# opendilab/LightZero

Hardware: NVIDIA H100
Metric: MCTS simulations/sec (batched search+infer) (higher is better)
Workload: dtype f32 (fp16x2-split tensor MMAs, fp32 accumulate)

## Files before the change

lightzero_b200/csrc/conv_tc.cu:

```cuda
#include <math.h>
#include <stdlib.h>
#include <string.h>

#include <algorithm>

#include "conv_tc.cuh"
#include "tc_ptx.cuh"

namespace lz {

constexpr int kCvConsumers = 256, kCvThreads = kCvConsumers + 32;
constexpr int kCvStages = 4;

struct CvBars {
    uint64_t full[kCvStages], empty[kCvStages];
    uint64_t in_full;
};

struct CvGeom {
    int nbands, rin, m_lo, mcount, NT, PR;
    size_t plane, part, phase, in_bytes, tap_bytes, smem;
};

__host__ __device__ inline CvGeom cv_geom(const ConvTc &p)
// ... 47 lines not shown
        mbar_init(&bars->in_full, 1);
        fence_mbar_init();
    }
    __syncthreads();

    if (warp == kCvConsumers / 32) {
        if (lane == 0) {
            const int grow0 = rin0 + 1;
            const int ncopy = min(g.rin, p.in.plane_rows - grow0);
            const uint32_t bytes = (uint32_t)ncopy * 16u;
            mbar_expect_tx(&bars->in_full, bytes * (uint32_t)(nimg * p.in.nphase * 2 * kg_in));
            for (int k = 0; k < nimg; ++k)
                for (int f = 0; f < p.in.nphase; ++f)
                    for (int part = 0; part < 2; ++part)
                        for (int kg = 0; kg < kg_in; ++kg) {
                            const unsigned char *src = p.in.base + (size_t)(img0 + k) * p.in.img_stride + f * p.in.phase_stride +
                                                       part * p.in.part_stride + ((size_t)kg * p.in.plane_rows + grow0) * 16;
                            unsigned char *dst = in_s + f * g.phase + part * g.part + kg * g.plane + (size_t)k * g.rin * 16;
                            bulk_g2s(dst, src, bytes, &bars->in_full);
                        }
            for (int n = 0; n < 9 * g.NT; ++n) {
                const int st = n % nstages, tap = n % 9;
                if (n >= nstages) mbar_wait(&bars->empty[st], ((n / nstages) - 1) & 1);
                mbar_expect_tx(&bars->full[st], (uint32_t)g.tap_bytes);
                bulk_g2s(ring + st * g.tap_bytes, p.w + (size_t)tap * g.tap_bytes, (uint32_t)g.tap_bytes, &bars->full[st]);
            }
        }
        return;
    }

    const int wg = warp >> 2;
    const uint32_t plane16 = (uint32_t)(g.plane >> 4);
    const uint64_t a_desc0 = make_desc(smem_u32(in_s), plane16, 8);
    const uint64_t b_desc0 = make_desc(smem_u32(ring), 2 * N, 8);
    const uint32_t b_lo16 = (uint32_t)N;
    const uint32_t a_lo16 = (uint32_t)(g.part >> 4);
    const int nks = kg_in / 2;
    const int yend = min(y0 + p.band_h, H);
    const int qc = 2 * (lane & 3);
    mbar_wait(&bars->in_full, 0);
    for (int t = 0; t < g.NT; ++t) {
        float acc[N / 2];
#pragma unroll
        for (int i = 0; i < N / 2; ++i) acc[i] = 0.0f;
        for (int tap = 0; tap < 9; ++tap) {
            const int n = t * 9 + tap, st = n % nstages;
            mbar_wait(&bars->full[st], (n / nstages) & 1);
            const uint64_t b0 = b_desc0 + (uint64_t)((st * g.tap_bytes) >> 4);
            const uint64_t a0 = a_desc0 + (uint64_t)((p.tap_phase[tap] * g.phase) >> 4) + (uint64_t)(g.m_lo + p.tap_shift[tap] + t * 128 + wg * 64);
            wg_fence();
            for (int ks = 0; ks < nks; ++ks) {
                wgmma_f16<N>(acc, a0 + ks * 2 * plane16, b0 + ks * 4 * N);
                if (npass == 3) {
                    wgmma_f16<N>(acc, a0 + ks * 2 * plane16, b0 + b_lo16 + ks * 4 * N);
                    wgmma_f16<N>(acc, a0 + a_lo16 + ks * 2 * plane16, b0 + ks * 4 * N);
                }
            }
            wg_commit();
            if (tap > 0) {
                wg_wait<1>();
                __syncwarp();
                if (lane == 0) mbar_arrive(&bars->empty[(n - 1) % nstages]);
            }
        }
        wg_wait<0>();
        __syncwarp();
        if (lane == 0) mbar_arrive(&bars->empty[(t * 9 + 8) % nstages]);

#pragma unroll
        for (int hr = 0; hr < 2; ++hr) {
            const int m = g.m_lo + t * 128 + wg * 64 + 16 * (warp & 3) + (lane >> 2) + 8 * hr;
            const int k = m / g.rin;
            const int rho = rin0 + (m - k * g.rin);
            const int yy = rho / pitch - 1, xx = rho - (yy + 1) * pitch;
            const bool in_band = (k < nimg) && (rho >= pitch) && (yy >= y0) && (yy < yend);
            const bool valid = in_band && (xx < W);
#pragma unroll
            for (int j = 0; j < N / 8; ++j) {
                const int col = 8 * j + qc;
                const int grp = (N == 128) ? (col >> 6) : 0;
                const int c = col - grp * 64;
                const Tcl &o = p.out[grp];
                const bool relu = p.relu[grp] != 0;
                size_t obase = 0;
                bool do_write = in_band;
                if (in_band) {
                    if (o.nphase == 1) {
                        obase = (size_t)(img0 + k) * o.img_stride + (size_t)(rho + 1) * 16;
                    } else if (valid) {
                        const int ph = (yy & 1) * 2 + (xx & 1);
                        const int rho2 = ((yy >> 1) + 1) * o.pitch + (xx >> 1);
                        obase = (size_t)(img0 + k) * o.img_stride + ph * o.phase_stride + (size_t)(rho2 + 1) * 16;
                    } else {
                        do_write = false;
                    }
                }
                float v0 = fmaf(acc[4 * j + 2 * hr], __ldg(p.scale + col), __ldg(p.shift + col));
                float v1 = fmaf(acc[4 * j + 2 * hr + 1], __ldg(p.scale + col + 1), __ldg(p.shift + col + 1));
                if (p.res.base && grp == 0 && valid) {
                    const unsigned char *rp = p.res.base + (size_t)(img0 + k) * p.res.img_stride +
                                              ((size_t)(c >> 3) * p.res.plane_rows + rho + 1) * 16 + (c & 7) * 2;
                    const float2 a = __half22float2(*reinterpret_cast<const __half2 *>(rp));
                    const float2 b = __half22float2(*reinterpret_cast<const __half2 *>(rp + p.res.part_stride));
                    v0 += a.x + b.x;
                    v1 += a.y + b.y;
                }
                v0 = valid ? (relu ? fmaxf(v0, 0.0f) : v0) : 0.0f;
                v1 = valid ? (relu ? fmaxf(v1, 0.0f) : v1) : 0.0f;
                if (do_write) {
                    unsigned char *op = o.base + obase + (size_t)(c >> 3) * o.plane_rows * 16 + (c & 7) * 2;
                    store_split2(op, op + o.part_stride, v0, v1);
                }
            }
        }
    }
}

__device__ __forceinline__ void tcl_load8(const Tcl &t, int img, int kg, int rho, float (&v)[8])
{
    const unsigned char *pp = t.base + (size_t)img * t.img_stride + ((size_t)kg * t.plane_rows + rho + 1) * 16;
    const uint4 rh = __ldg(reinterpret_cast<const uint4 *>(pp));
    const uint4 rl = __ldg(reinterpret_cast<const uint4 *>(pp + t.part_stride));
    const __half2 *hh = reinterpret_cast<const __half2 *>(&rh), *hl = reinterpret_cast<const __half2 *>(&rl);
#pragma unroll
    for (int j = 0; j < 4; ++j) {
        const float2 a = __half22float2(hh[j]), b = __half22float2(hl[j]);
        v[2 * j] = a.x + b.x;
        v[2 * j + 1] = a.y + b.y;
    }
}

__global__ void k_pool_tcl(Tcl in, Tcl out, float *out_nchw, int B, int Hout)
{
    const int kgs = in.C / 8;
    const size_t n = (size_t)B * kgs * Hout * Hout;
    for (size_t i = blockIdx.x * (size_t)blockDim.x + threadIdx.x; i < n; i += (size_t)gridDim.x * blockDim.x) {
        const int xo = (int)(i % Hout), yo = (int)((i / Hout) % Hout);
        const int kg = (int)((i / ((size_t)Hout * Hout)) % kgs), img = (int)(i / ((size_t)Hout * Hout * kgs));
        float s[8];
#pragma unroll
        for (int j = 0; j < 8; ++j) s[j] = 0.0f;
#pragma unroll
        for (int ky = 0; ky < 3; ++ky) {
            const int yy = 2 * yo + ky - 1;
            if (yy < 0 || yy >= in.H) continue;
#pragma unroll
            for (int kx = 0; kx < 3; ++kx) {
                const int xx = 2 * xo + kx - 1;
                if (xx < 0 || xx >= in.W) continue;
                float v[8];
                tcl_load8(in, img, kg, (yy + 1) * in.pitch + xx, v);
#pragma unroll
                for (int j = 0; j < 8; ++j) s[j] += v[j];
            }
        }
#pragma unroll
        for (int j = 0; j < 8; ++j) s[j] = s[j] / 9.0f;
        if (out_nchw) {
#pragma unroll
            for (int j = 0; j < 8; ++j) out_nchw[((size_t)img * in.C + kg * 8 + j) * Hout * Hout + yo * Hout + xo] = s[j];
        } else {
            unsigned char *op = out.base + (size_t)img * out.img_stride + ((size_t)kg * out.plane_rows + (yo + 1) * out.pitch + xo + 1) * 16;
            store_split8(op, op + out.part_stride, s);
        }
    }
}

int conv_tc_prepare_launch()
{
    const int big = 227 * 1024;
    LZ_CUDA_CHECK(cudaFuncSetAttribute(k_conv_tc<32>, cudaFuncAttributeMaxDynamicSharedMemorySize, big));
    LZ_CUDA_CHECK(cudaFuncSetAttribute(k_conv_tc<64>, cudaFuncAttributeMaxDynamicSharedMemorySize, big));
    LZ_CUDA_CHECK(cudaFuncSetAttribute(k_conv_tc<128>, cudaFuncAttributeMaxDynamicSharedMemorySize, big));
    return LZ_OK;
}

int conv_tc_launch(const ConvTc &p, cudaStream_t s)
{
    const CvGeom g = cv_geom(p);
    LZ_REQUIRE(g.smem <= 227 * 1024, LZ_EINVAL, "conv_tc: band needs %zu B shared memory", g.smem);
    LZ_REQUIRE(g.tap_bytes <= 16384 && (p.in.C % 16) == 0, LZ_EINVAL, "conv_tc: unsupported channel counts");
    const int groups = (p.B + p.G - 1) / p.G;
    const int grid = groups * g.nbands;
    switch (p.N) {
        case 32: k_conv_tc<32><<<grid, kCvThreads, g.smem, s>>>(p); break;
        case 64: k_conv_tc<64><<<grid, kCvThreads, g.smem, s>>>(p); break;
        case 128: k_conv_tc<128><<<grid, kCvThreads, g.smem, s>>>(p); break;
        default: LZ_REQUIRE(false, LZ_EINVAL, "conv_tc: N must be 32, 64 or 128");
    }
    LZ_KERNEL_CHECK();
    return LZ_OK;
}

size_t conv_tc_packed_bytes(int cin, int ncols) { return (size_t)9 * 2 * (cin / 8) * ncols * 16; }

float conv_tc_pack(const float *w, int cin, int cout, int ncols, int col0, unsigned char *dst)
{
    float mx = 0.0f;
    for (size_t i = 0; i < (size_t)cout * cin * 9; ++i) mx = std::max(mx, fabsf(w[i]));
    int e = 0;
    if (mx > 0.0f) frexpf(mx, &e);
    const float scale = ldexpf(1.0f, 13 - e);
    const size_t tap_halves = (size_t)2 * (cin / 8) * ncols * 8, part_halves = (size_t)ncols * 8;
    __half *h = reinterpret_cast<__half *>(dst);
    for (int t = 0; t < 9; ++t)
        for (int co = 0; co < cout; ++co)
            for (int ci = 0; ci < cin; ++ci) {
                const float sv = w[((size_t)co * cin + ci) * 9 + t] * scale;
                const __half hi = __float2half_rn(sv);
                const __half lo = __float2half_rn(sv - __half2float(hi));
                const size_t off = (size_t)t * tap_halves + ((size_t)(ci / 8) * 2 * ncols + col0 + co) * 8 + (ci % 8);
                h[off] = hi;
                h[off + part_halves] = lo;
            }
    return scale;
}

int pool_tcl_launch(const Tcl &in, const Tcl &out, int B, cudaStream_t s)
{
    const size_t n = (size_t)B * (in.C / 8) * out.H * out.W;
    k_pool_tcl<<<(int)std::min<size_t>((n + 255) / 256, kNumSMs * 32), 256, 0, s>>>(in, out, nullptr, B, out.H);
    LZ_KERNEL_CHECK();
    return LZ_OK;
}

int pool_tcl_to_nchw_launch(const Tcl &in, float *out, int B, int Hout, cudaStream_t s)
{
    const size_t n = (size_t)B * (in.C / 8) * Hout * Hout;
    Tcl dummy = in;
    k_pool_tcl<<<(int)std::min<size_t>((n + 255) / 256, kNumSMs * 32), 256, 0, s>>>(in, dummy, out, B, Hout);
    LZ_KERNEL_CHECK();
    return LZ_OK;
}

}
```

lightzero_b200/csrc/conv_tc.cuh:

```cuda
#pragma once
#include "lz_common.cuh"

namespace lz {

struct Tcl {
    unsigned char *base;
    size_t img_stride, phase_stride, part_stride;
    int plane_rows;
    int C, H, W, pitch;
    int nphase;
};

inline Tcl make_tcl(unsigned char *base, int C, int H, int W, int nphase)
{
    Tcl t;
    t.base = base; t.C = C; t.H = H; t.W = W; t.pitch = W + 1; t.nphase = nphase;
    t.plane_rows = (H + 2) * (W + 1) + 2;
    t.part_stride = (size_t)(C / 8) * t.plane_rows * 16;
    t.phase_stride = 2 * t.part_stride;
    t.img_stride = t.phase_stride * nphase;
    return t;
}
inline size_t tcl_bytes(int B, int C, int H, int W, int nphase)
{
    return (size_t)B * nphase * 2 * (C / 8) * ((size_t)(H + 2) * (W + 1) + 2) * 16;
}

struct ConvTc {
    Tcl in;
    Tcl out[2];
    Tcl res;
    const unsigned char *w;
    const float *scale, *shift;
    int tap_phase[9], tap_shift[9];
    int relu[2];
    int N;
    int G, band_h;
    int stages;
    int B, npass;
};

int conv_tc_prepare_launch();
int conv_tc_launch(const ConvTc &p, cudaStream_t s);
float conv_tc_pack(const float *w_torch, int cin, int cout, int ncols, int col0, unsigned char *dst);
size_t conv_tc_packed_bytes(int cin, int ncols);

int pool_tcl_launch(const Tcl &in, const Tcl &out, int B, cudaStream_t s);
int pool_tcl_to_nchw_launch(const Tcl &in, float *out, int B, int Hout, cudaStream_t s);

}
```

lightzero_b200/csrc/model.cu:

```cuda
#include <math.h>
#include <string.h>

#include <algorithm>

#include "model.cuh"
#include "tc_ptx.cuh"

namespace lz {

constexpr int kActFloats = kC * kP;
constexpr int kHFlatMax = 16 * kP;
constexpr int kKpad = 608;

template <int W>
__device__ __forceinline__ void heads_and_outputs(const NetDev &net, float *actA, float *actB, float *hrew,
                                                  float *wstage, bool with_reward, int B, float *o_reward,
                                                  float *o_value, float *o_policy, float *o_reward_logits,
                                                  float *o_value_logits)
{
    const int w = threadIdx.x >> 5, lane = threadIdx.x & 31;
    const int A = net.A, Apad = (A + 31) & ~31;
    float *lg_rew = actB;
    float *lg_val = actB + W * kKpad;
    float *lg_pol = actB + 2 * W * kKpad;
// ... 374 lines not shown
        }
        return tc_launch(m->tc_rec, t, s);
    }
    switch (pick_W(io.B)) {
        case 8: return launch_recurrent<8>(m->net, io, s);
        case 4: return launch_recurrent<4>(m->net, io, s);
        case 2: return launch_recurrent<2>(m->net, io, s);
        default: return launch_recurrent<1>(m->net, io, s);
    }
}

static int launch_convg(const ConvG &L, const float *in, float *out, const float *res, int relu, int B, cudaStream_t s,
                        const Tcl *tcl = nullptr, const uint8_t *in_u8 = nullptr)
{
    Tcl t;
    memset(&t, 0, sizeof(t));
    if (tcl) t = *tcl;
    const int cic = std::min(8, L.cin);
    const int rows_out_max = std::min(L.hout, 127 / L.wout + 2);
    const int nrows_max = (rows_out_max - 1) * L.stride + 3;
    const int pitch = L.win + 2;
    const size_t smem = ((((size_t)cic * nrows_max * pitch + 3) & ~(size_t)3) + (size_t)cic * 288) * sizeof(float);
    dim3 grid(ceil_div(L.hout * L.wout, 128), L.cout / 32, B);
    LZ_REQUIRE(smem <= 200 * 1024, LZ_EINVAL, "conv tower stage needs %zu B shared memory", smem);
    if (L.stride == 1) k_conv3x3_generic<1><<<grid, 128, smem, s>>>(L, in, out, res, relu, cic, nrows_max, t, in_u8);
    else k_conv3x3_generic<2><<<grid, 128, smem, s>>>(L, in, out, res, relu, cic, nrows_max, t, in_u8);
    LZ_KERNEL_CHECK();
    return LZ_OK;
}

static int launch_pool(const float *in, float *out, int planes, int hin, int hout, cudaStream_t s)
{
    const size_t n = (size_t)planes * hout * hout;
    int blocks = (int)std::min<size_t>((n + 255) / 256, kNumSMs * 16);
    k_avgpool3s2<<<blocks, 256, 0, s>>>(in, out, planes, hin, hin, hout, hout);
    LZ_KERNEL_CHECK();
    return LZ_OK;
}

static int reserve_tc_skip(lz_model *m, int B)
{
    if (m->kind != 0 || B <= m->tc_skip_B) return LZ_OK;
    ++m->generation;
    cudaFree(m->tc_skip);
    m->tc_skip = nullptr; m->tc_skip_B = 0;
    int rc = dev_alloc(&m->tc_skip, (size_t)kActFloats * B);
    if (rc != LZ_OK) return rc;
    m->tc_skip_B = B;
    return LZ_OK;
}

int model_reserve(lz_model *m, int B)
{
    {
        int rc = reserve_tc_skip(m, B);
        if (rc != LZ_OK) return rc;
    }
    if (m->kind == 0 && m->cfg.efficientzero && B > m->ez_B) {
        ++m->generation;
        cudaFree(m->ez_feat); cudaFree(m->ez_htmp);
        m->ez_feat = m->ez_htmp = nullptr;
        int rc = dev_alloc(&m->ez_feat, (size_t)B * m->cfg.reward_head_channels * kP);
        if (rc == LZ_OK) rc = dev_alloc(&m->ez_htmp, (size_t)B * m->cfg.lstm_hidden_size);
        if (rc != LZ_OK) return rc;
        m->ez_B = B;
    }
    if (m->kind == 1 || B <= m->ws_B) return LZ_OK;
    ++m->generation;
    size_t per_root = 0;
    for (const ConvG &L : m->tower) per_root = std::max(per_root, (size_t)L.cout * L.hout * L.wout);
    per_root = std::max(per_root, (size_t)kActFloats);
    for (int i = 0; i < 3; ++i) {
        if (m->ws[i]) cudaFree(m->ws[i]);
        m->ws[i] = nullptr;
        int rc = dev_alloc(&m->ws[i], per_root * B);
        if (rc != LZ_OK) return rc;
    }
    m->ws_floats = per_root * B;
    m->ws_B = B;
    {
        const int h1 = m->tower[0].hout, h2 = m->tower[3].hout, h3 = (h2 - 1) / 2 + 1, c2 = kC / 2;
        const size_t bT = tcl_bytes(B, c2, h1, h1, 1), bT2 = tcl_bytes(B, c2, h1 / 2, h1 / 2, 4);
        const size_t bU = tcl_bytes(B, kC, h2, h2, 1), bV = tcl_bytes(B, kC, h3, h3, 1);
        const size_t total = 2 * bT + bT2 + 3 * bU + 3 * bV;
        if (m->tws) cudaFree(m->tws);
        m->tws = nullptr;
        int rc = dev_alloc(&m->tws, total);
        if (rc != LZ_OK) return rc;
        LZ_CUDA_CHECK(cudaMemset(m->tws, 0, total));
        m->tws_bytes = total;
        unsigned char *q = m->tws;
        m->T0 = make_tcl(q, c2, h1, h1, 1); q += bT;
        m->T1 = make_tcl(q, c2, h1, h1, 1); q += bT;
        m->T2 = make_tcl(q, c2, h1 / 2, h1 / 2, 4); q += bT2;
        m->U0 = make_tcl(q, kC, h2, h2, 1); q += bU;
        m->U1 = make_tcl(q, kC, h2, h2, 1); q += bU;
        m->U2 = make_tcl(q, kC, h2, h2, 1); q += bU;
        m->V0 = make_tcl(q, kC, h3, h3, 1); q += bV;
        m->V1 = make_tcl(q, kC, h3, h3, 1); q += bV;
        m->V2 = make_tcl(q, kC, h3, h3, 1); q += bV;
    }
    return LZ_OK;
}

static void pick_band(ConvTc &p)
{
    const int H = p.in.H, pitch = p.in.pitch, kg = p.in.C / 8;
    double best = -1.0;
    int best_h = 1, best_g = 1, best_st = 4;
    for (int G = 1; G <= 4; ++G)
        for (int bh = (G > 1 ? H : 1); bh <= H; ++bh)
            for (int st = 2; st <= 4; st += 2) {
                const int rin = (bh + 2) * pitch + 2, mcount = (G - 1) * rin + bh * pitch, NT = (mcount + 127) / 128;
                int PR = pitch + 1 + NT * 128 + pitch + 2;
                if (PR < G * rin) PR = G * rin;
                const size_t smem = (((size_t)PR * 16 * kg * 2 * p.in.nphase + 127) & ~(size_t)127) + st * (size_t)2 * kg * p.N * 16 + 1024;
                if (smem > 227 * 1024) continue;
                const int nb = (H + bh - 1) / bh;
                double score = (double)(G * H * (pitch - 1)) / ((double)nb * NT * 128);
                if (p.N <= 64 && smem <= 113 * 1024) score *= 1.35;
                score *= (st == 4) ? 1.0 : 0.97;
                if (score > best + 1e-9) { best = score; best_h = bh; best_g = G; best_st = st; }
            }
    p.band_h = best_h;
    p.G = best_g;
    p.stages = best_st;
}

static int tower_tc_run(lz_model *m, int B, const float *d_obs, float *pre_latent, cudaStream_t s, const uint8_t *d_obs_u8 = nullptr)
{
    int rc;
    const int npass = (m->math == 1) ? 3 : 1;
    const ConvG &S0 = m->tower[0];
    if (m->stem_valid) {
        const int rows_per_cta = std::max(1, 256 / S0.wout);
        const size_t smem = (size_t)4 * (2 * rows_per_cta + 1) * (S0.win + 4) * sizeof(float);
        dim3 grid(ceil_div(S0.hout, rows_per_cta), B);
        const StemP &P = *reinterpret_cast<const StemP *>(m->stem_params.data());
        if (d_obs_u8) k_stem4_tcl<true><<<grid, 256, smem, s>>>(P, nullptr, d_obs_u8, S0.hin, S0.win, S0.hout, S0.wout, rows_per_cta, m->T0);
        else k_stem4_tcl<false><<<grid, 256, smem, s>>>(P, d_obs, nullptr, S0.hin, S0.win, S0.hout, S0.wout, rows_per_cta, m->T0);
        LZ_KERNEL_CHECK();
    } else if ((rc = launch_convg(S0, d_obs, nullptr, nullptr, 1, B, s, &m->T0, d_obs_u8))) return rc;
    auto run = [&](ConvTc p, const Tcl &in, const Tcl &o0, const Tcl *o1, const Tcl *res) {
        p.in = in; p.out[0] = o0;
        if (o1) p.out[1] = *o1;
        if (res) p.res = *res; else p.res.base = nullptr;
        p.B = B; p.npass = npass;
        return conv_tc_launch(p, s);
    };
    if ((rc = run(m->tower_tc[0], m->T0, m->T1, nullptr, nullptr))) return rc;
    if ((rc = run(m->tower_tc[1], m->T1, m->T2, nullptr, &m->T0))) return rc;
    if ((rc = run(m->tower_tc[2], m->T2, m->U0, &m->U1, nullptr))) return rc;
    if ((rc = run(m->tower_tc[3], m->U0, m->U2, nullptr, &m->U1))) return rc;
    if ((rc = run(m->tower_tc[4], m->U2, m->U0, nullptr, nullptr))) return rc;
    if ((rc = run(m->tower_tc[5], m->U0, m->U1, nullptr, &m->U2))) return rc;
    if ((rc = pool_tcl_launch(m->U1, m->V0, B, s))) return rc;
    if ((rc = run(m->tower_tc_rb3[0], m->V0, m->V1, nullptr, nullptr))) return rc;
    if ((rc = run(m->tower_tc_rb3[1], m->V1, m->V2, nullptr, &m->V0))) return rc;
    return pool_tcl_to_nchw_launch(m->V2, pre_latent, B, kHW, s);
}

int model_initial_tower(lz_model *m, int B, const float *d_obs, float *pre_latent, cudaStream_t s, const uint8_t *d_obs_u8)
{
    LZ_REQUIRE(m->kind == 0 && m->math != 0 && m->cfg.obs_h != 64, LZ_ESTATE, "model_initial_tower: tensor-core conv model only");
    LZ_REQUIRE(B <= m->ws_B, LZ_ESTATE, "model_initial_tower: workspace sized for %d roots, got %d", m->ws_B, B);
    return tower_tc_run(m, B, d_obs, pre_latent, s, d_obs_u8);
}

int model_initial_tail(lz_model *m, int B, const float *pre_latent, const TailIO &io_in, cudaStream_t s)
{
    TcIO t;
    memset(&t, 0, sizeof(t));
    t.B = B; t.npass = (m->math == 1) ? 3 : 1;
    t.latent_base = pre_latent; t.latent_out = io_in.latent; t.latent_out2 = io_in.latent2;
    t.value = io_in.value; t.policy_logits = io_in.policy_logits; t.value_logits = io_in.value_logits;
    LZ_REQUIRE(B <= m->tc_skip_B, LZ_ESTATE, "model_initial_tail: scratch sized for %d roots, got %d (model_reserve)", m->tc_skip_B, B);
    t.skip_scratch = m->tc_skip;
    return tc_launch(m->tc_tail, t, s);
}

int model_initial(lz_model *m, int B, const float *d_obs, const TailIO &io_in, cudaStream_t s)
{
    if (m->kind == 1) return mlp_initial(m, B, d_obs, io_in, s);
    LZ_REQUIRE(B <= m->ws_B, LZ_ESTATE, "model_initial: workspace sized for %d roots, got %d (call model_reserve outside capture)", m->ws_B, B);
    float *a = m->ws[0], *b = m->ws[1], *c = m->ws[2];
    const std::vector<ConvG> &T = m->tower;
    int rc;
    if (m->math != 0 && m->cfg.obs_h != 64) {
        if ((rc = tower_tc_run(m, B, d_obs, a, s))) return rc;
        return model_initial_tail(m, B, a, io_in, s);
    }
    if ((rc = launch_convg(T[0], d_obs, a, nullptr, 1, B, s))) return rc;
    if ((rc = launch_convg(T[1], a, b, nullptr, 1, B, s))) return rc;
    if ((rc = launch_convg(T[2], b, c, a, 1, B, s))) return rc;
    if ((rc = launch_convg(T[3], c, a, nullptr, 0, B, s))) return rc;
    if ((rc = launch_convg(T[4], c, b, nullptr, 1, B, s))) return rc;
    if ((rc = launch_convg(T[5], b, c, a, 1, B, s))) return rc;
    if ((rc = launch_convg(T[6], c, a, nullptr, 1, B, s))) return rc;
    if ((rc = launch_convg(T[7], a, b, c, 1, B, s))) return rc;
    const int h2 = T[7].hout, h3 = (h2 - 1) / 2 + 1;
    if ((rc = launch_pool(b, a, B * kC, h2, h3, s))) return rc;
    if ((rc = launch_convg(T[8], a, b, nullptr, 1, B, s))) return rc;
    if ((rc = launch_convg(T[9], b, c, a, 1, B, s))) return rc;
    const float *pre = c;
    if (m->cfg.obs_h != 64) {
        const int h4 = (h3 - 1) / 2 + 1;
        if ((rc = launch_pool(c, a, B * kC, h3, h4, s))) return rc;
        pre = a;
    }
    if (m->math != 0) return model_initial_tail(m, B, pre, io_in, s);
    TailIO io = io_in;
    io.B = B;
    io.pre_latent = pre;
    switch (pick_W(B)) {
        case 8: return launch_tail<8>(m->net, io, s);
        case 4: return launch_tail<4>(m->net, io, s);
        case 2: return launch_tail<2>(m->net, io, s);
        default: return launch_tail<1>(m->net, io, s);
    }
}

struct Packer {
    std::vector<float> host;
    size_t add(const std::vector<float> &v)
    {
        while (host.size() % 4) host.push_back(0.0f);
        size_t off = host.size();
        host.insert(host.end(), v.begin(), v.end());
        return off;
    }
};

static const std::vector<float> *find(lz_model *m, const std::string &name, size_t expect)
{
    auto it = m->tensors.find(name);
    if (it == m->tensors.end()) { set_error("lz_model_finalize: missing tensor '%s'", name.c_str()); return nullptr; }
    if (expect && it->second.size() != expect) {
        set_error("lz_model_finalize: tensor '%s' has %zu elements, expected %zu", name.c_str(), it->second.size(), expect);
        return nullptr;
    }
    return &it->second;
}
// ... 50 lines not shown
    if (!W0 || !B0 || !W3 || !B3) return false;
    if (!fold_bn(m, fc + ".1", hid, s2, t2)) return false;
    for (int j = 0; j < hid; ++j) t2[j] += s2[j] * (*B0)[j];
    const int nin = hc * Pix;
    std::vector<float> fc1((size_t)nin * hid), fc2((size_t)hid * K);
    for (int j = 0; j < hid; ++j)
        for (int i = 0; i < nin; ++i) fc1[(size_t)i * hid + j] = (*W0)[(size_t)j * nin + i];
    for (int k = 0; k < K; ++k)
        for (int j = 0; j < hid; ++j) fc2[(size_t)j * K + k] = (*W3)[(size_t)k * hid + j];
    o.w1 = P.add(*w1); o.s1 = P.add(s1); o.t1 = P.add(t1); o.fc1 = P.add(fc1);
    o.s2 = P.add(s2); o.t2 = P.add(t2); o.fc2 = P.add(fc2); o.b2 = P.add(*B3);
    o.hc = hc; o.hid = hid; o.K = K;
    return true;
}

static int pack_tower_tc(lz_model *m)
{
    const std::string R = "representation_network.downsample_net.";
    const int c2 = kC / 2;
    const int h1 = m->tower[0].hout, h2 = m->tower[3].hout, h3 = (h2 - 1) / 2 + 1;
    struct Item { std::string w, bn; int cin, cout; };
    const Item items[9] = {
        {R + "resblocks1.0.conv1.0.weight", R + "resblocks1.0.conv1.1", c2, c2},
        {R + "resblocks1.0.conv2.0.weight", R + "resblocks1.0.conv2.1", c2, c2},
        {R + "downsample_block.conv1.0.weight", R + "downsample_block.conv1.1", c2, kC},
        {R + "downsample_block.conv3.0.weight", "", c2, kC},
        {R + "downsample_block.conv2.0.weight", R + "downsample_block.conv2.1", kC, kC},
        {R + "resblocks2.0.conv1.0.weight", R + "resblocks2.0.conv1.1", kC, kC},
        {R + "resblocks2.0.conv2.0.weight", R + "resblocks2.0.conv2.1", kC, kC},
        {R + "resblocks3.0.conv1.0.weight", R + "resblocks3.0.conv1.1", kC, kC},
        {R + "resblocks3.0.conv2.0.weight", R + "resblocks3.0.conv2.1", kC, kC},
    };
    struct Lay { int it0, it1, cin, N; };
    const Lay lays[8] = {{0, -1, c2, c2}, {1, -1, c2, c2}, {2, 3, c2, 2 * kC}, {4, -1, kC, kC},
                         {5, -1, kC, kC}, {6, -1, kC, kC}, {7, -1, kC, kC}, {8, -1, kC, kC}};
    size_t wbytes = 0;
    for (const Lay &l : lays) wbytes += conv_tc_packed_bytes(l.cin, l.N);
    size_t tab_off = (wbytes + 255) & ~(size_t)255;
    std::vector<unsigned char> host(tab_off + 8 * 2 * 128 * sizeof(float), 0);
    float *tab = reinterpret_cast<float *>(host.data() + tab_off);
    size_t woff[8], off = 0;
    for (int li = 0; li < 8; ++li) {
        const Lay &l = lays[li];
        woff[li] = off;
        float *scale = tab + li * 256, *shift = scale + 128;
        for (int part = 0; part < 2; ++part) {
            const int it = part == 0 ? l.it0 : l.it1;
            if (it < 0) continue;
            const Item &I = items[it];
            auto w = find(m, I.w, (size_t)I.cout * I.cin * 9);
            if (!w) return LZ_EINVAL;
            std::vector<float> sc(I.cout, 1.0f), sh(I.cout, 0.0f);
            if (!I.bn.empty() && !fold_bn(m, I.bn, I.cout, sc, sh)) return LZ_EINVAL;
            const int col0 = part * kC;
            const float ws = conv_tc_pack(w->data(), I.cin, I.cout, l.N, col0, host.data() + off);
            for (int k = 0; k < I.cout; ++k) { scale[col0 + k] = sc[k] / ws; shift[col0 + k] = sh[k]; }
        }
        off += conv_tc_packed_bytes(l.cin, l.N);
    }
    if (m->d_tower) cudaFree(m->d_tower);
    m->d_tower = nullptr;
    int rc = dev_alloc(&m->d_tower, host.size());
    if (rc != LZ_OK) return rc;
    LZ_CUDA_CHECK(cudaMemcpy(m->d_tower, host.data(), host.size(), cudaMemcpyHostToDevice));
    const float *dtab = reinterpret_cast<const float *>(m->d_tower + tab_off);
    auto base = [&](int li, int N, int H, int nphase_in, int C_in) {
        ConvTc p;
        memset(&p, 0, sizeof(p));
        p.w = m->d_tower + woff[li];
        p.scale = dtab + li * 256; p.shift = p.scale + 128;
        p.N = N; p.relu[0] = 1; p.relu[1] = 0;
        p.in = make_tcl(nullptr, C_in, H, H, nphase_in);
        for (int t = 0; t < 9; ++t) {
            const int ky = t / 3, kx = t % 3;
            if (nphase_in == 1) { p.tap_phase[t] = 0; p.tap_shift[t] = (ky - 1) * p.in.pitch + (kx - 1); }
            else {
                p.tap_phase[t] = (((ky + 1) & 1) * 2) + ((kx + 1) & 1);
                p.tap_shift[t] = (ky == 0 ? -p.in.pitch : 0) + (kx == 0 ? -1 : 0);
            }
        }
        pick_band(p);
        return p;
    };
    m->tower_tc[0] = base(0, c2, h1, 1, c2);
    m->tower_tc[1] = base(1, c2, h1, 1, c2);
    m->tower_tc[2] = base(2, 2 * kC, h2, 4, c2);
    m->tower_tc[3] = base(3, kC, h2, 1, kC);
    m->tower_tc[4] = base(4, kC, h2, 1, kC);
    m->tower_tc[5] = base(5, kC, h2, 1, kC);
    m->tower_tc_rb3[0] = base(6, kC, h3, 1, kC);
    m->tower_tc_rb3[1] = base(7, kC, h3, 1, kC);
    return conv_tc_prepare_launch();
}

static int pack_tc(lz_model *m, const NetDev &net)
{
    const lz_model_config &c = m->cfg;
    const int A = c.action_space_size, n = c.num_res_blocks;
    const int nconv = 1 + 6 * n;
    const size_t conv_bytes = (size_t)tc_conv_layout_bytes();
    const size_t off_convw = 0;
    const size_t off_headw = off_convw + conv_bytes * nconv;
    const size_t off_bn = off_headw + tc_head_layout_bytes();
    const size_t off_headbn = off_bn + (size_t)nconv * 128 * 4;
    const size_t off_abias = off_headbn + 96 * 4;
    const std::string fc_names[3] = {"dynamics_network.fc_reward_head", "prediction_network.fc_value", "prediction_network.fc_policy"};
    const Head *fc_heads[3] = {&net.reward, &net.value, &net.policy};
    size_t fc_off2[3];
    size_t off_fc = (off_abias + (size_t)A * kC * kP * 4 + 127) & ~(size_t)127;
    const size_t off_fc0 = off_fc;
    off_fc += (size_t)18 * 12288;
    for (int h = 0; h < 3; ++h) {
        fc_off2[h] = off_fc - off_fc0;
        if (fc_heads[h]->hid > 0) off_fc += (size_t)((fc_heads[h]->K + 127) / 128) * 16384;
    }
    const size_t total = off_fc;
    std::vector<unsigned char> host(total, 0);
    float *bn = reinterpret_cast<float *>(host.data() + off_bn);
    float *head_bn = reinterpret_cast<float *>(host.data() + off_headbn);
    float *abias = reinterpret_cast<float *>(host.data() + off_abias);

    std::vector<std::pair<std::string, std::string>> convs;
    const std::string D = "dynamics_network.", Q = "prediction_network.", R = "representation_network.";
    convs.push_back({D + "conv.weight", D + "norm_common"});
    for (const std::string &pre : {D, Q, R})
        for (int i = 0; i < n; ++i) {
            const std::string b = pre + "resblocks." + std::to_string(i);
            convs.push_back({b + ".conv1.0.weight", b + ".conv1.1"});
            convs.push_back({b + ".conv2.0.weight", b + ".conv2.1"});
        }
    for (int ci = 0; ci < nconv; ++ci) {
        const int cin_total = (ci == 0) ? kC + A : kC;
        auto w = find(m, convs[ci].first, (size_t)kC * cin_total * 9);
        std::vector<float> scale, shift;
        if (!w || !fold_bn(m, convs[ci].second, kC, scale, shift)) return LZ_EINVAL;
        const float ws = tc_pack_conv3(w->data(), cin_total, kC, host.data() + off_convw + conv_bytes * ci);
        for (int k = 0; k < kC; ++k) { bn[ci * 128 + k] = scale[k] / ws; bn[ci * 128 + 64 + k] = shift[k]; }
        if (ci == 0) {
            for (int a = 0; a < A; ++a)
                for (int co = 0; co < kC; ++co)
                    for (int y = 0; y < kHW; ++y)
                        for (int x = 0; x < kHW; ++x) {
                            float acc = 0.0f;
                            for (int ky = 0; ky < 3; ++ky)
                                for (int kx = 0; kx < 3; ++kx) {
                                    const int yy = y + ky - 1, xx = x + kx - 1;
                                    if (yy < 0 || yy >= kHW || xx < 0 || xx >= kHW) continue;
                                    acc += (*w)[((size_t)co * cin_total + kC + a) * 9 + ky * 3 + kx];
                                }
                            abias[(((size_t)a * 16 + co / 4) * kP + y * kHW + x) * 4 + co % 4] = acc * scale[co];
                        }
        }
    }
    struct HD { std::string conv, norm; int hc, nco, co_off; size_t hi, lo; int bn_off; };
    const HD heads[3] = {
        {D + "conv1x1_reward", D + "norm_reward", c.reward_head_channels, 16, 0, off_headw, off_headw + 2048, 0},
        {Q + "conv1x1_value", Q + "norm_value", c.value_head_channels, 32, 0, off_headw + 4096, off_headw + 8192, 32},
        {Q + "conv1x1_policy", Q + "norm_policy", c.policy_head_channels, 32, 16, off_headw + 4096, off_headw + 8192, 64},
    };
    for (const HD &h : heads) {
        auto w1 = find(m, h.conv + ".weight", (size_t)h.hc * kC), b1 = find(m, h.conv + ".bias", h.hc);
        std::vector<float> s1, t1;
        if (!w1 || !b1 || !fold_bn(m, h.norm, h.hc, s1, t1)) return LZ_EINVAL;
        const float ws = tc_pack_conv1(w1->data(), h.hc, h.nco, h.co_off, host.data() + h.hi, host.data() + h.lo);
        for (int i = 0; i < h.hc; ++i) {
            head_bn[h.bn_off + i] = s1[i] / ws;
            head_bn[h.bn_off + 16 + i] = t1[i] + s1[i] * (*b1)[i];
        }
    }
    float fc1_inv[3] = {1.0f, 1.0f, 1.0f}, fc2_inv[3] = {1.0f, 1.0f, 1.0f};
    for (int h = 0; h < 3; ++h) {
        const Head &H = *fc_heads[h];
        if (H.hid <= 0) continue;
        const int nin = H.hc * kP;
// ... 385 lines not shown
```

lightzero_b200/csrc/model.cuh:

```cuda
#pragma once
#include <map>
#include <string>
#include <vector>

#include "lz_common.cuh"
#include "net6.cuh"
#include "net_tc.cuh"
#include "conv_tc.cuh"
#include "ez.cuh"

namespace lz {

constexpr int kMaxResBlocks = 4;

struct NetDev {
    Conv3 dyn_conv;
    Conv3 dyn_res[2 * kMaxResBlocks];
    Conv3 pred_res[2 * kMaxResBlocks];
    Conv3 rep_res[2 * kMaxResBlocks];
    Head reward, value, policy;
    int nres;
    int A;
    float support_min, support_step;
};

struct ConvG {
    const float *w;
    const float *scale, *shift;
    int cin, cout, stride, hin, win, hout, wout;
};

struct Dense {
    const float *wt, *scale, *shift;
    int in, out, act, nact;
};

struct MlpNet {
    Dense e0, e1;
    Dense d1a, d1b, d2a, d2b;
    Dense r0, r1, pc0, pc1, v0, v1, p0, p1;
    const float *ln_w, *ln_b;
    int latent, obs_dim, A, res;
    float support_min, support_step;
};

struct RecIO {
    int B;
    const float *latent_base;
    const int *ix;
    size_t slot_stride;
    const int *action;
    float *next_latent;
    float *reward, *value;
    float *policy_logits;
    float *reward_logits, *value_logits;
    float *skip_scratch;
    const float *h_base, *c_base;
    size_t hslot_stride;
    float *h_out, *c_out;
    const int *is_reset;
};

struct TailIO {
    int B;
    const float *pre_latent;
    float *latent;
    float *latent2;
    float *value;
    float *policy_logits;
    float *value_logits;
};

}

struct lz_model {
    int kind;
    lz::EzNet ez;
    float *ez_feat, *ez_htmp;
    int ez_B;
    unsigned char *d_ez_wtc;
    int latent_floats;
    lz_mlp_config mcfg;
    lz::MlpNet mlp;
    lz_model_config cfg;
    std::map<std::string, std::vector<float>> tensors;
    bool finalized;
    float *d_weights;
    size_t n_weight_floats;
    lz::NetDev net;
    std::vector<lz::ConvG> tower;
    std::vector<float> stem_params;
    int stem_valid;
    int hw, P, K;
    int math;
    unsigned char *d_tc;
    lz::TcNet tc_rec, tc_tail;
    float *tc_skip;
    int tc_skip_B;
    unsigned char *d_tower;
    lz::ConvTc tower_tc[7];
    lz::ConvTc tower_tc_rb3[2];
    unsigned char *tws;
    size_t tws_bytes;
    lz::Tcl T0, T1, T2, U0, U1, U2, V0, V1, V2;
    float *ws[3];
    size_t ws_floats;
    int ws_B;
    unsigned long long generation;
};

namespace lz {
int model_recurrent(lz_model *m, const RecIO &io, cudaStream_t s);
int model_initial(lz_model *m, int B, const float *d_obs, const TailIO &io, cudaStream_t s);
int model_initial_tower(lz_model *m, int B, const float *d_obs, float *pre_latent, cudaStream_t s, const uint8_t *d_obs_u8 = nullptr);
int model_initial_tail(lz_model *m, int B, const float *pre_latent, const TailIO &io, cudaStream_t s);
int model_reserve(lz_model *m, int B);
int mlp_recurrent(lz_model *m, const RecIO &io, cudaStream_t s);
int mlp_initial(lz_model *m, int B, const float *d_obs, const TailIO &io, cudaStream_t s);
int mlp_finalize(lz_model *m);
}
```

Baseline: 4.394 million.

## Fuse residual block conv pairs into one kernel with shared-memory intermediate

Adds a resblock kernel that runs both 3x3 convolutions of a residual block in one launch. It keeps the intermediate activation and the residual input in shared memory, recomputing a one-row halo per band. Three conv-pair launches in the representation tower are replaced, which removes global round-trips and launches. The cost is redundant halo compute, a tighter shared-memory budget that may force smaller groups or bands, and dropped support for phase-split output in the generic conv kernel.

```diff
diff --git a/lightzero_b200/csrc/conv_tc.cu b/lightzero_b200/csrc/conv_tc.cu
--- a/lightzero_b200/csrc/conv_tc.cu
+++ b/lightzero_b200/csrc/conv_tc.cu
@@ -153,19 +153,6 @@
                 const int c = col - grp * 64;
                 const Tcl &o = p.out[grp];
                 const bool relu = p.relu[grp] != 0;
-                size_t obase = 0;
-                bool do_write = in_band;
-                if (in_band) {
-                    if (o.nphase == 1) {
-                        obase = (size_t)(img0 + k) * o.img_stride + (size_t)(rho + 1) * 16;
-                    } else if (valid) {
-                        const int ph = (yy & 1) * 2 + (xx & 1);
-                        const int rho2 = ((yy >> 1) + 1) * o.pitch + (xx >> 1);
-                        obase = (size_t)(img0 + k) * o.img_stride + ph * o.phase_stride + (size_t)(rho2 + 1) * 16;
-                    } else {
-                        do_write = false;
-                    }
-                }
                 float v0 = fmaf(acc[4 * j + 2 * hr], __ldg(p.scale + col), __ldg(p.shift + col));
                 float v1 = fmaf(acc[4 * j + 2 * hr + 1], __ldg(p.scale + col + 1), __ldg(p.shift + col + 1));
                 if (p.res.base && grp == 0 && valid) {
@@ -178,8 +165,225 @@
                 }
                 v0 = valid ? (relu ? fmaxf(v0, 0.0f) : v0) : 0.0f;
                 v1 = valid ? (relu ? fmaxf(v1, 0.0f) : v1) : 0.0f;
+                if (in_band) {
+                    unsigned char *op = o.base + (size_t)(img0 + k) * o.img_stride + ((size_t)(c >> 3) * o.plane_rows + rho + 1) * 16 + (c & 7) * 2;
+                    store_split2(op, op + o.part_stride, v0, v1);
+                }
+            }
+        }
+    }
+}
+
+constexpr int kRbChunks = 16;
+
+struct RbBars {
+    uint64_t full[kCvStages], empty[kCvStages];
+    uint64_t chunk[kRbChunks];
+};
+
+struct RbGeom {
+    int nbands, S, m_lo, NT1, NT2, PR, nchunk;
+    size_t plane, part, buf, tap_bytes, smem;
+};
+
+__host__ __device__ inline RbGeom rb_geom(const ResBlockTc &p)
+{
+    RbGeom g;
+    const int H = p.in.H, pitch = p.in.pitch, kg = p.in.C / 8;
+    g.nbands = (H + p.band_h - 1) / p.band_h;
+    g.S = (p.band_h + 4) * pitch + 2;
+    g.m_lo = pitch + 1;
+    g.NT1 = ((p.G - 1) * g.S + (p.band_h + 2) * pitch + 127) / 128;
+    g.NT2 = ((p.G - 1) * g.S + p.band_h * pitch + 127) / 128;
+    g.PR = p.G * g.S;
+    g.nchunk = (g.PR + 127) / 128;
+    g.plane = (size_t)g.PR * 16;
+    g.part = (size_t)kg * g.plane;
+    g.buf = (2 * g.part + 127) & ~(size_t)127;
+    g.tap_bytes = (size_t)2 * kg * p.in.C * 16;
+    g.smem = 2 * g.buf + p.stages * g.tap_bytes + 1024;
+    return g;
+}
+
+template <int N>
+__device__ __forceinline__ void rb_tiles(float (&acc)[2][N / 2], bool two, uint64_t a_desc0, int row0, const ResBlockTc &p,
+                                         const RbGeom &g, uint64_t b_desc0, RbBars *bars, int n0, int lane)
+{
+    const uint32_t plane16 = (uint32_t)(g.plane >> 4), a_lo16 = (uint32_t)(g.part >> 4), b_lo16 = (uint32_t)N;
+    const int nstages = p.stages;
+#pragma unroll
+    for (int s = 0; s < 2; ++s)
+#pragma unroll
+        for (int i = 0; i < N / 2; ++i) acc[s][i] = 0.0f;
+    for (int tap = 0; tap < 9; ++tap) {
+        const int n = n0 + tap, st = n % nstages;
+        mbar_wait(&bars->full[st], (n / nstages) & 1);
+        const uint64_t b0 = b_desc0 + (uint64_t)((st * g.tap_bytes) >> 4);
+        const uint64_t a0 = a_desc0 + (uint64_t)(row0 + p.tap_shift[tap]);
+        wg_fence();
+        for (int ks = 0; ks < N / 16; ++ks) {
+#pragma unroll
+            for (int s = 0; s < 2; ++s) {
+                if (s == 1 && !two) break;
+                const uint64_t as = a0 + s * 128 + ks * 2 * plane16;
+                wgmma_f16<N>(acc[s], as, b0 + ks * 4 * N);
+                if (p.npass == 3) {
+                    wgmma_f16<N>(acc[s], as, b0 + b_lo16 + ks * 4 * N);
+                    wgmma_f16<N>(acc[s], as + a_lo16, b0 + ks * 4 * N);
+                }
+            }
+        }
+        wg_commit();
+        if (tap > 0) {
+            wg_wait<1>();
+            __syncwarp();
+            if (lane == 0) mbar_arrive(&bars->empty[(n - 1) % nstages]);
+        }
+    }
+    wg_wait<0>();
+    __syncwarp();
+    if (lane == 0) mbar_arrive(&bars->empty[(n0 + 8) % nstages]);
+}
+
+template <int N>
+__global__ void __launch_bounds__(kCvThreads, 1) k_resblock_tc(ResBlockTc p)
+{
+    extern __shared__ __align__(1024) unsigned char smem[];
+    const RbGeom g = rb_geom(p);
+    unsigned char *in_s = smem, *mid_s = smem + g.buf, *ring = smem + 2 * g.buf;
+    RbBars *bars = reinterpret_cast<RbBars *>(ring + p.stages * g.tap_bytes);
+    const int nstages = p.stages;
+    const int tid = threadIdx.x, warp = __shfl_sync(0xffffffffu, tid >> 5, 0), lane = tid & 31;
+    const int pitch = p.in.pitch, H = p.in.H, W = p.in.W, kg_in = N / 8;
+    const int group = blockIdx.x / g.nbands, band = blockIdx.x - group * g.nbands;
+    const int img0 = group * p.G, nimg = min(p.G, p.B - img0);
+    const int y0 = band * p.band_h;
+    const int np1 = (g.NT1 + 1) / 2, ntaps = 9 * (np1 + (g.NT2 + 1) / 2);
+
+    if (tid == 0) {
+        for (int i = 0; i < kCvStages; ++i) { mbar_init(&bars->full[i], 1); mbar_init(&bars->empty[i], kCvConsumers / 32); }
+        for (int c = 0; c < g.nchunk; ++c) mbar_init(&bars->chunk[c], 1);
+        fence_mbar_init();
+    }
+    __syncthreads();
+
+    if (warp == kCvConsumers / 32) {
+        if (lane == 0) {
+            auto load_tap = [&](int n) {
+                const int st = n % nstages, tap = n % 9;
+                if (n >= nstages) mbar_wait(&bars->empty[st], ((n / nstages) - 1) & 1);
+                mbar_expect_tx(&bars->full[st], (uint32_t)g.tap_bytes);
+                bulk_g2s(ring + st * g.tap_bytes, p.w[n >= 9 * np1] + (size_t)tap * g.tap_bytes, (uint32_t)g.tap_bytes, &bars->full[st]);
+            };
+            for (int n = 0; n < nstages; ++n) load_tap(n);
+            const int g0 = (y0 - 1) * pitch;
+            const int r0 = max(0, -g0), r1 = min(g.S, p.in.plane_rows - g0);
+            for (int c = 0; c < g.nchunk; ++c) {
+                uint32_t rows = 0;
+                for (int k = 0; k < nimg; ++k) rows += (uint32_t)max(0, min(k * g.S + r1, c * 128 + 128) - max(k * g.S + r0, c * 128));
+                mbar_expect_tx(&bars->chunk[c], rows * 16u * (uint32_t)(2 * kg_in));
+                for (int k = 0; k < nimg; ++k) {
+                    const int lo = max(k * g.S + r0, c * 128), hi = min(k * g.S + r1, c * 128 + 128);
+                    if (hi <= lo) continue;
+                    for (int part = 0; part < 2; ++part)
+                        for (int kg = 0; kg < kg_in; ++kg) {
+                            const unsigned char *src = p.in.base + (size_t)(img0 + k) * p.in.img_stride + part * p.in.part_stride +
+                                                       ((size_t)kg * p.in.plane_rows + g0 + lo - k * g.S) * 16;
+                            bulk_g2s(in_s + part * g.part + kg * g.plane + (size_t)lo * 16, src, (uint32_t)(hi - lo) * 16u, &bars->chunk[c]);
+                        }
+                }
+            }
+            for (int n = nstages; n < ntaps; ++n) load_tap(n);
+        }
+        return;
+    }
+
+    const int wg = warp >> 2;
+    const uint32_t plane16 = (uint32_t)(g.plane >> 4);
+    const uint64_t in_desc = make_desc(smem_u32(in_s), plane16, 8), mid_desc = make_desc(smem_u32(mid_s), plane16, 8);
+    const uint64_t b_desc0 = make_desc(smem_u32(ring), 2 * N, 8);
+    const int qc = 2 * (lane & 3);
+    if (tid < 2 * kg_in) *reinterpret_cast<uint4 *>(mid_s + tid * g.plane) = make_uint4(0u, 0u, 0u, 0u);
+
+    int ready = 0;
+    for (int t = 0; t < g.NT1; t += 2) {
+        const bool two = t + 1 < g.NT1;
+        const int need = min(g.nchunk, (t * 128 + 256 + 2 * pitch + 1) / 128 + 1);
+        for (; ready < need; ++ready) mbar_wait(&bars->chunk[ready], 0);
+        float acc[2][N / 2];
+        rb_tiles<N>(acc, two, in_desc, g.m_lo + t * 128 + wg * 64, p, g, b_desc0, bars, t / 2 * 9, lane);
+#pragma unroll
+        for (int e = 0; e < 4; ++e) {
+            const int s = e >> 1, hr = e & 1;
+            if (s == 1 && !two) break;
+            const int m = g.m_lo + (t + s) * 128 + wg * 64 + 16 * (warp & 3) + (lane >> 2) + 8 * hr;
+            const int i = m - pitch;
+            const int k = m / g.S;
+            const int rho = (y0 - 1) * pitch - 1 + (m - k * g.S);
+            const int yy = rho / pitch - 1, xx = rho - (yy + 1) * pitch;
+            const bool valid = (k < nimg) && (rho >= pitch) && (yy >= y0 - 1) && (yy <= y0 + p.band_h) && (yy < H) && (xx < W);
+            if (i >= g.PR) continue;
+#pragma unroll
+            for (int j = 0; j < N / 8; ++j) {
+                const int col = 8 * j + qc;
+                float v0 = fmaf(acc[s][4 * j + 2 * hr], __ldg(p.scale[0] + col), __ldg(p.shift[0] + col));
+                float v1 = fmaf(acc[s][4 * j + 2 * hr + 1], __ldg(p.scale[0] + col + 1), __ldg(p.shift[0] + col + 1));
+                v0 = valid ? fmaxf(v0, 0.0f) : 0.0f;
+                v1 = valid ? fmaxf(v1, 0.0f) : 0.0f;
+                unsigned char *op = mid_s + (size_t)(col >> 3) * g.plane + (size_t)i * 16 + (col & 7) * 2;
+                store_split2(op, op + g.part, v0, v1);
+            }
+        }
+    }
+    for (; ready < g.nchunk; ++ready) mbar_wait(&bars->chunk[ready], 0);
+    fence_proxy_async();
+    asm volatile("bar.sync 1, %0;\n" ::"n"(kCvConsumers) : "memory");
+
+    const int yend = min(y0 + p.band_h, H);
+    for (int t = 0; t < g.NT2; t += 2) {
+        const bool two = t + 1 < g.NT2;
+        float acc[2][N / 2];
+        rb_tiles<N>(acc, two, mid_desc, g.m_lo + t * 128 + wg * 64, p, g, b_desc0, bars, (np1 + t / 2) * 9, lane);
+#pragma unroll
+        for (int e = 0; e < 4; ++e) {
+            const int s = e >> 1, hr = e & 1;
+            if (s == 1 && !two) break;
+            const int m = g.m_lo + (t + s) * 128 + wg * 64 + 16 * (warp & 3) + (lane >> 2) + 8 * hr;
+            const int k = m / g.S;
+            const int rho = y0 * pitch - 1 + (m - k * g.S);
+            const int yy = rho / pitch - 1, xx = rho - (yy + 1) * pitch;
+            const bool in_band = (k < nimg) && (rho >= pitch) && (yy >= y0) && (yy < yend);
+            const bool valid = in_band && (xx < W);
+            const Tcl &o = p.out;
+            size_t obase = 0;
+            bool do_write = in_band;
+            if (in_band) {
+                if (o.nphase == 1) {
+                    obase = (size_t)(img0 + k) * o.img_stride + (size_t)(rho + 1) * 16;
+                } else if (valid) {
+                    const int ph = (yy & 1) * 2 + (xx & 1);
+                    const int rho2 = ((yy >> 1) + 1) * o.pitch + (xx >> 1);
+                    obase = (size_t)(img0 + k) * o.img_stride + ph * o.phase_stride + (size_t)(rho2 + 1) * 16;
+                } else {
+                    do_write = false;
+                }
+            }
+#pragma unroll
+            for (int j = 0; j < N / 8; ++j) {
+                const int col = 8 * j + qc;
+                float v0 = fmaf(acc[s][4 * j + 2 * hr], __ldg(p.scale[1] + col), __ldg(p.shift[1] + col));
+                float v1 = fmaf(acc[s][4 * j + 2 * hr + 1], __ldg(p.scale[1] + col + 1), __ldg(p.shift[1] + col + 1));
+                if (valid) {
+                    const unsigned char *rp = in_s + (size_t)(col >> 3) * g.plane + (size_t)(m + pitch) * 16 + (col & 7) * 2;
+                    const float2 a = __half22float2(*reinterpret_cast<const __half2 *>(rp));
+                    const float2 b = __half22float2(*reinterpret_cast<const __half2 *>(rp + g.part));
+                    v0 += a.x + b.x;
+                    v1 += a.y + b.y;
+                }
+                v0 = valid ? fmaxf(v0, 0.0f) : 0.0f;
+                v1 = valid ? fmaxf(v1, 0.0f) : 0.0f;
                 if (do_write) {
-                    unsigned char *op = o.base + obase + (size_t)(c >> 3) * o.plane_rows * 16 + (c & 7) * 2;
+                    unsigned char *op = o.base + obase + (size_t)(col >> 3) * o.plane_rows * 16 + (col & 7) * 2;
                     store_split2(op, op + o.part_stride, v0, v1);
                 }
             }
@@ -240,9 +444,10 @@
 int conv_tc_prepare_launch()
 {
     const int big = 227 * 1024;
-    LZ_CUDA_CHECK(cudaFuncSetAttribute(k_conv_tc<32>, cudaFuncAttributeMaxDynamicSharedMemorySize, big));
     LZ_CUDA_CHECK(cudaFuncSetAttribute(k_conv_tc<64>, cudaFuncAttributeMaxDynamicSharedMemorySize, big));
     LZ_CUDA_CHECK(cudaFuncSetAttribute(k_conv_tc<128>, cudaFuncAttributeMaxDynamicSharedMemorySize, big));
+    LZ_CUDA_CHECK(cudaFuncSetAttribute(k_resblock_tc<32>, cudaFuncAttributeMaxDynamicSharedMemorySize, big));
+    LZ_CUDA_CHECK(cudaFuncSetAttribute(k_resblock_tc<64>, cudaFuncAttributeMaxDynamicSharedMemorySize, big));
     return LZ_OK;
 }
 
@@ -251,13 +456,47 @@
     const CvGeom g = cv_geom(p);
     LZ_REQUIRE(g.smem <= 227 * 1024, LZ_EINVAL, "conv_tc: band needs %zu B shared memory", g.smem);
     LZ_REQUIRE(g.tap_bytes <= 16384 && (p.in.C % 16) == 0, LZ_EINVAL, "conv_tc: unsupported channel counts");
+    LZ_REQUIRE(p.out[0].nphase == 1 && (p.N < 128 || p.out[1].nphase == 1), LZ_EINVAL, "conv_tc: phase-split output is not supported");
     const int groups = (p.B + p.G - 1) / p.G;
     const int grid = groups * g.nbands;
     switch (p.N) {
-        case 32: k_conv_tc<32><<<grid, kCvThreads, g.smem, s>>>(p); break;
         case 64: k_conv_tc<64><<<grid, kCvThreads, g.smem, s>>>(p); break;
         case 128: k_conv_tc<128><<<grid, kCvThreads, g.smem, s>>>(p); break;
-        default: LZ_REQUIRE(false, LZ_EINVAL, "conv_tc: N must be 32, 64 or 128");
+        default: LZ_REQUIRE(false, LZ_EINVAL, "conv_tc: N must be 64 or 128");
+    }
+    LZ_KERNEL_CHECK();
+    return LZ_OK;
+}
+
+int resblock_tc_plan(ResBlockTc &p)
+{
+    const int H = p.in.H, W = p.in.W;
+    ResBlockTc q = p;
+    double best = -1.0;
+    for (int G = 1; G <= 4; ++G)
+        for (int bh = (G > 1 ? H : 1); bh <= H; ++bh)
+            for (int st = 2; st <= 4; st += 2) {
+                q.G = G; q.band_h = bh; q.stages = st;
+                const RbGeom g = rb_geom(q);
+                if (g.smem > 227 * 1024 || g.nchunk > kRbChunks) continue;
+                double score = (double)(2 * G * H * W) / ((double)g.nbands * (g.NT1 + g.NT2) * 128);
+                score *= (st == 4) ? 1.0 : 0.97;
+                if (score > best + 1e-9) { best = score; p.G = G; p.band_h = bh; p.stages = st; }
+            }
+    LZ_REQUIRE(best > 0.0, LZ_EINVAL, "resblock_tc: no band of a %dx%d, %d-channel block fits shared memory", H, W, p.in.C);
+    return LZ_OK;
+}
+
+int resblock_tc_launch(const ResBlockTc &p, cudaStream_t s)
+{
+    const RbGeom g = rb_geom(p);
+    LZ_REQUIRE(g.smem <= 227 * 1024 && g.nchunk <= kRbChunks, LZ_EINVAL, "resblock_tc: band needs %zu B shared memory", g.smem);
+    LZ_REQUIRE(p.in.nphase == 1 && p.out.C == p.in.C, LZ_EINVAL, "resblock_tc: unsupported input / output layout");
+    const int grid = (p.B + p.G - 1) / p.G * g.nbands;
+    switch (p.in.C) {
+        case 32: k_resblock_tc<32><<<grid, kCvThreads, g.smem, s>>>(p); break;
+        case 64: k_resblock_tc<64><<<grid, kCvThreads, g.smem, s>>>(p); break;
+        default: LZ_REQUIRE(false, LZ_EINVAL, "resblock_tc: channels must be 32 or 64");
     }
     LZ_KERNEL_CHECK();
     return LZ_OK;
diff --git a/lightzero_b200/csrc/conv_tc.cuh b/lightzero_b200/csrc/conv_tc.cuh
--- a/lightzero_b200/csrc/conv_tc.cuh
+++ b/lightzero_b200/csrc/conv_tc.cuh
@@ -40,8 +40,21 @@
     int B, npass;
 };
 
+struct ResBlockTc {
+    Tcl in;
+    Tcl out;
+    const unsigned char *w[2];
+    const float *scale[2], *shift[2];
+    int tap_shift[9];
+    int G, band_h;
+    int stages;
+    int B, npass;
+};
+
 int conv_tc_prepare_launch();
 int conv_tc_launch(const ConvTc &p, cudaStream_t s);
+int resblock_tc_plan(ResBlockTc &p);
+int resblock_tc_launch(const ResBlockTc &p, cudaStream_t s);
 float conv_tc_pack(const float *w_torch, int cin, int cout, int ncols, int col0, unsigned char *dst);
 size_t conv_tc_packed_bytes(int cin, int ncols);
 
diff --git a/lightzero_b200/csrc/model.cu b/lightzero_b200/csrc/model.cu
--- a/lightzero_b200/csrc/model.cu
+++ b/lightzero_b200/csrc/model.cu
@@ -480,7 +480,7 @@
         const int h1 = m->tower[0].hout, h2 = m->tower[3].hout, h3 = (h2 - 1) / 2 + 1, c2 = kC / 2;
         const size_t bT = tcl_bytes(B, c2, h1, h1, 1), bT2 = tcl_bytes(B, c2, h1 / 2, h1 / 2, 4);
         const size_t bU = tcl_bytes(B, kC, h2, h2, 1), bV = tcl_bytes(B, kC, h3, h3, 1);
-        const size_t total = 2 * bT + bT2 + 3 * bU + 3 * bV;
+        const size_t total = bT + bT2 + 3 * bU + 2 * bV;
         if (m->tws) cudaFree(m->tws);
         m->tws = nullptr;
         int rc = dev_alloc(&m->tws, total);
@@ -489,14 +489,12 @@
         m->tws_bytes = total;
         unsigned char *q = m->tws;
         m->T0 = make_tcl(q, c2, h1, h1, 1); q += bT;
-        m->T1 = make_tcl(q, c2, h1, h1, 1); q += bT;
-        m->T2 = make_tcl(q, c2, h1 / 2, h1 / 2, 4); q += bT2;
+        m->T1 = make_tcl(q, c2, h1 / 2, h1 / 2, 4); q += bT2;
         m->U0 = make_tcl(q, kC, h2, h2, 1); q += bU;
         m->U1 = make_tcl(q, kC, h2, h2, 1); q += bU;
         m->U2 = make_tcl(q, kC, h2, h2, 1); q += bU;
         m->V0 = make_tcl(q, kC, h3, h3, 1); q += bV;
         m->V1 = make_tcl(q, kC, h3, h3, 1); q += bV;
-        m->V2 = make_tcl(q, kC, h3, h3, 1); q += bV;
     }
     return LZ_OK;
 }
@@ -546,16 +544,18 @@
         p.B = B; p.npass = npass;
         return conv_tc_launch(p, s);
     };
-    if ((rc = run(m->tower_tc[0], m->T0, m->T1, nullptr, nullptr))) return rc;
-    if ((rc = run(m->tower_tc[1], m->T1, m->T2, nullptr, &m->T0))) return rc;
-    if ((rc = run(m->tower_tc[2], m->T2, m->U0, &m->U1, nullptr))) return rc;
-    if ((rc = run(m->tower_tc[3], m->U0, m->U2, nullptr, &m->U1))) return rc;
-    if ((rc = run(m->tower_tc[4], m->U2, m->U0, nullptr, nullptr))) return rc;
-    if ((rc = run(m->tower_tc[5], m->U0, m->U1, nullptr, &m->U2))) return rc;
-    if ((rc = pool_tcl_launch(m->U1, m->V0, B, s))) return rc;
-    if ((rc = run(m->tower_tc_rb3[0], m->V0, m->V1, nullptr, nullptr))) return rc;
-    if ((rc = run(m->tower_tc_rb3[1], m->V1, m->V2, nullptr, &m->V0))) return rc;
-    return pool_tcl_to_nchw_launch(m->V2, pre_latent, B, kHW, s);
+    auto rb = [&](ResBlockTc p, const Tcl &in, const Tcl &out) {
+        p.in = in; p.out = out;
+        p.B = B; p.npass = npass;
+        return resblock_tc_launch(p, s);
+    };
+    if ((rc = rb(m->tower_rb[0], m->T0, m->T1))) return rc;
+    if ((rc = run(m->tower_tc[0], m->T1, m->U0, &m->U1, nullptr))) return rc;
+    if ((rc = run(m->tower_tc[1], m->U0, m->U2, nullptr, &m->U1))) return rc;
+    if ((rc = rb(m->tower_rb[1], m->U2, m->U0))) return rc;
+    if ((rc = pool_tcl_launch(m->U0, m->V0, B, s))) return rc;
+    if ((rc = rb(m->tower_rb[2], m->V0, m->V1))) return rc;
+    return pool_tcl_to_nchw_launch(m->V1, pre_latent, B, kHW, s);
 }
 
 int model_initial_tower(lz_model *m, int B, const float *d_obs, float *pre_latent, cudaStream_t s, const uint8_t *d_obs_u8)
@@ -772,14 +772,21 @@
         pick_band(p);
         return p;
     };
-    m->tower_tc[0] = base(0, c2, h1, 1, c2);
-    m->tower_tc[1] = base(1, c2, h1, 1, c2);
-    m->tower_tc[2] = base(2, 2 * kC, h2, 4, c2);
-    m->tower_tc[3] = base(3, kC, h2, 1, kC);
-    m->tower_tc[4] = base(4, kC, h2, 1, kC);
-    m->tower_tc[5] = base(5, kC, h2, 1, kC);
-    m->tower_tc_rb3[0] = base(6, kC, h3, 1, kC);
-    m->tower_tc_rb3[1] = base(7, kC, h3, 1, kC);
+    m->tower_tc[0] = base(2, 2 * kC, h2, 4, c2);
+    m->tower_tc[1] = base(3, kC, h2, 1, kC);
+    auto block = [&](ResBlockTc &p, int li, int C, int H) {
+        memset(&p, 0, sizeof(p));
+        for (int c = 0; c < 2; ++c) {
+            p.w[c] = m->d_tower + woff[li + c];
+            p.scale[c] = dtab + (li + c) * 256; p.shift[c] = p.scale[c] + 128;
+        }
+        p.in = make_tcl(nullptr, C, H, H, 1);
+        for (int t = 0; t < 9; ++t) p.tap_shift[t] = (t / 3 - 1) * p.in.pitch + (t % 3 - 1);
+        return resblock_tc_plan(p);
+    };
+    if ((rc = block(m->tower_rb[0], 0, c2, h1))) return rc;
+    if ((rc = block(m->tower_rb[1], 4, kC, h2))) return rc;
+    if ((rc = block(m->tower_rb[2], 6, kC, h3))) return rc;
     return conv_tc_prepare_launch();
 }
 
diff --git a/lightzero_b200/csrc/model.cuh b/lightzero_b200/csrc/model.cuh
--- a/lightzero_b200/csrc/model.cuh
+++ b/lightzero_b200/csrc/model.cuh
@@ -98,11 +98,11 @@
     float *tc_skip;
     int tc_skip_B;
     unsigned char *d_tower;
-    lz::ConvTc tower_tc[7];
-    lz::ConvTc tower_tc_rb3[2];
+    lz::ConvTc tower_tc[2];
+    lz::ResBlockTc tower_rb[3];
     unsigned char *tws;
     size_t tws_bytes;
-    lz::Tcl T0, T1, T2, U0, U1, U2, V0, V1, V2;
+    lz::Tcl T0, T1, U0, U1, U2, V0, V1;
     float *ws[3];
     size_t ws_floats;
     int ws_B;
```

Result: faster. 4.583 million, median of 6 (+4.3%).
